# jeuneS2/csolve

Measured on AMD Instinct MI355X. Metric: constraint propagations/sec + nodes/sec, queens-N, 1/2/4/8 MI355X, higher is better.
Workload: dtype int32

## Files before the change

csolve_amd/_lib.py:

```python
from __future__ import annotations

import ctypes as C
import os
import re

_HERE = os.path.dirname(os.path.abspath(__file__))
LIB_PATH = os.environ.get("CSOLVE_HIP_LIB") or os.path.join(_HERE, "libcsolve_hip.so")
HEADER_PATH = os.path.join(os.path.dirname(_HERE), "include", "csolve_gpu.h")


class CsolveError(RuntimeError):
    def __init__(self, code: int, message: str):
        super().__init__(f"csolve_gpu error {code}: {message}")
        self.code = code


class Val(C.Structure):
    _fields_ = [("lo", C.c_int32), ("hi", C.c_int32)]


class Node(C.Structure):
    _fields_ = [("var", C.c_int32), ("lo", C.c_int32), ("hi", C.c_int32), ("parent", C.c_int32)]


# ... 173 lines not shown
    L.csgpu_search_drain_solutions_device.argtypes = [vp, vp, i64, C.POINTER(i64), vp]
    L.csgpu_search_pending_solutions.argtypes = [vp, C.POINTER(i64), C.POINTER(i64)]
    L.csgpu_propagate_one.argtypes = [vp, vp, Node, vp, C.POINTER(Result)]
    L.csgpu_propagate_one_traced.argtypes = [vp, vp, Node, vp, C.POINTER(Result), vp, i32, C.POINTER(i32)]
    L.csgpu_propagate_one_causes.argtypes = [vp, vp, Node, vp, C.POINTER(Result), vp, i32, C.POINTER(i32)]
    L.csgpu_propagate_values.argtypes = [vp, vp, i32, vp, i32, vp, vp]
    L.csgpu_model_root_propagate_limit.argtypes = [vp, i64, C.POINTER(i32), C.POINTER(i32)]
    L.csgpu_propagate_one_chain.argtypes = [vp, vp, Node, C.POINTER(i32), C.POINTER(i32), vp, i32, C.POINTER(i32)]
    L.csgpu_search_set_strategy.argtypes = [vp, C.c_int, C.c_int]
    L.csgpu_search_set_restart_on_improvement.argtypes = [vp, C.c_int]
    L.csgpu_internal_plan_symbol.argtypes = [vp, C.c_int, C.c_char_p, C.c_size_t]
    L.csgpu_solve_many.argtypes = [vp, vp, i64, C.POINTER(ManyOptions), vp, vp, vp]
    L.csgpu_internal_many_symbol.argtypes = [vp, C.c_char_p, C.c_size_t]
    L.csgpu_internal_many_waves.argtypes = [vp, i64]
    L.csgpu_internal_many_waves.restype = i64
    L.csgpu_internal_many_resume_symbol.argtypes = [vp, C.c_char_p, C.c_size_t]
    L.csgpu_many_checkpoint_bytes.argtypes = [vp]
    L.csgpu_many_checkpoint_bytes.restype = C.c_size_t
    L.csgpu_many_checkpoints_create.argtypes = [vp, i64, C.POINTER(vp)]
    L.csgpu_many_checkpoints_reset.argtypes = [vp, vp]
    L.csgpu_many_checkpoints_free.argtypes = [vp]
    L.csgpu_many_checkpoints_free.restype = None
    L.csgpu_solve_many_checkpointed.argtypes = [vp, vp, i64, C.POINTER(ManyOptions), vp, vp, vp, vp, vp]
    L.csgpu_solve_many_resume.argtypes = [vp, i64, C.POINTER(ManyOptions), vp, vp, vp, vp, vp]
    L.csgpu_many_checkpoint_states.argtypes = [vp, C.c_int32, vp, i64, C.POINTER(i64), vp]
    L.csgpu_solve_many_upto.argtypes = [vp, vp, i64, C.POINTER(ManyUptoOptions), vp, vp, vp]
    L.csgpu_solve_many_upto_checkpointed.argtypes = [vp, vp, i64, C.POINTER(ManyUptoOptions), vp, vp, vp, vp, vp]
    L.csgpu_solve_many_upto_resume.argtypes = [vp, i64, C.POINTER(ManyUptoOptions), vp, vp, vp, vp, vp]
    L.csgpu_internal_many_upto_symbol.argtypes = [vp, C.c_char_p, C.c_size_t]
    L.csgpu_solve_many_restarts.argtypes = [vp, vp, vp, i64, C.POINTER(ManyRestartOptions), vp, vp, vp, vp]
# ... 13 lines not shown
```

csolve_amd/csrc/cs_capi.hip:

```cpp
#include <hip/hip_runtime.h>
#include <chrono>

#include <dlfcn.h>
#include <stdarg.h>
#include <stdio.h>
#include <stdlib.h>
#include <string.h>

#include <mutex>

#include "../../include/csolve_gpu.h"
#include "cs_kernels.hip.h"
#include "cs_shave.hip.h"
#include "cs_step.hip.h"
#include "cs_dive.hip.h"
#include "cs_chain.hip.h"
#include "cs_internal.h"

static thread_local char g_err[512] = "";

static int set_err(int code, const char *fmt, ...) {
  va_list ap;
  va_start(ap, fmt);
  vsnprintf(g_err, sizeof g_err, fmt, ap);
// ... 50 lines not shown
  int not_root;
  int finalized;
  cs_dev_image *img;
  int *d_adj_off, *d_adj, *d_clause, *d_tree_off, *d_tnode, *d_tkid, *d_tree_want, *d_lit, *d_clause_by_kind;
  cs_tables tab;
  size_t slice;
  int has_tree_adj;
  int packed_bias;
  int packed_nw;
  int kernel_choice;
  cs_kernel_plan plan;
  void *d_adj_packed;
  int lds_adj_global;
  int k2_csz;
  int shave_static;
  int step_chunk_max;
  size_t k1_tab_bytes;
  int fb_words;
  size_t dense_bytes;
  void *d_dense_tab;
  void *d_packed_tab;
  int *d_root_lo;
  int *d_root_hi;
  void *d_many_stack;
  int64_t many_stack_waves;
  unsigned *d_many_tickets;
  int *d_sym_off;
  void *d_sym_packed;
  int n_cus;
  unsigned *d_tickets;
// ... 159 lines not shown
  (void)hipFree(m->d_lit);
  m->d_tree_want = NULL;
  m->d_lit = NULL;
  (void)hipFree(m->d_adj_packed);
  (void)hipFree(m->d_root_lo);
  (void)hipFree(m->d_root_hi);
  (void)hipFree(m->d_many_stack);
  (void)hipFree(m->d_many_tickets);
  m->d_root_hi = NULL;
  m->d_many_stack = NULL;
  m->d_many_tickets = NULL;
  m->many_stack_waves = 0;
  (void)hipFree(m->d_sym_off);
  (void)hipFree(m->d_sym_packed);
  (void)hipFree(m->d_dense_tab);
  (void)hipFree(m->d_packed_tab);
  m->d_packed_tab = NULL;
  (void)hipFree(m->d_tickets);
  m->d_tickets = NULL;
  m->ticket_slots = m->ticket_streams = m->ticket_reserved = 0;
  m->d_sym_off = NULL;
  m->d_sym_packed = NULL;
  m->d_dense_tab = NULL;
  m->d_adj_packed = NULL;
  m->d_root_lo = NULL;
  memset(&m->plan, 0, sizeof m->plan);
  m->fb_words = 0;
  (void)hipHostFree(m->h_one);
  m->h_one = NULL;
  (void)hipFree(m->d_adj_clause);
// ... 692 lines not shown
  const cs_model *h = m->host;
  if (!m->fb_words) return CSGPU_OK;
  const int n = h->n_vars, width = m->img->dense_width, slots = m->img->dense_slots;
  size_t bytes = 0;
  const int waves = dense_table_waves(m, &bytes);
  if (!waves) return CSGPU_OK;
  m->dense_bytes = bytes;
  int rc;
  if ((rc = upload(m->img->dense_tab, bytes, (int **)&m->d_dense_tab))) return rc;
  for (int variant = 0; variant < 4; variant++)
    if ((rc = plan_kernel(&m->plan.regs[variant], ne_regs_kernel(width, m->fb_words, n, variant & 1, variant >> 1), bytes, waves)))
      return rc;
  m->plan.full = n == cs_dense_strides(n) * CS_WAVE;
  if ((rc = plan_kernel(&m->plan.shave, ne_shave_kernel(width, n, slots, m->plan.full), bytes, waves))) return rc;
  const size_t table = (bytes + 15) & ~(size_t)15;
  if (table + (size_t)waves * 32 <= CS_CU_LDS &&
      (rc = plan_kernel(&m->plan.step_shave, step_shave_kernel(width, n, slots, m->plan.full), table + (size_t)waves * 32, waves)))
    return rc;
  if (table + CS_SHAVE_TRACE_LDS * 16 <= CS_CU_LDS) {
    if ((rc = plan_kernel(&m->plan.shave_trace, ne_shave_trace_kernel(width, n, slots), table + CS_SHAVE_TRACE_LDS * 16, waves)))
      return rc;
    m->plan.server = m->plan.shave_trace;
    m->plan.server.fn = shave_server_kernel(width, n, slots);
  }
  for (int family = 0; family < MANY_FAMILIES; family++)
    if ((rc = plan_kernel(&m->plan.dive[family], dive_kernel(family, width, n), table, waves))) return rc;
  {
    int *hi = (int *)malloc((size_t)n * sizeof(int));
    if (hi == NULL) return set_err(CSGPU_E_ARG, "out of memory");
    for (int32_t v = 0; v < n; v++) hi[v] = h->dom[v].hi;
// ... 131 lines not shown
  const void *fn = m->plan.dive[family].fn;
  const char *name = many_kernel_name[family];
  if (fn == NULL) return CSGPU_OK;
  Dl_info info;
  if (dladdr(fn, &info) == 0 || info.dli_sname == NULL || info.dli_saddr != fn)
    return set_err(CSGPU_E_STATE, "%s: the kernel handle has no dynamic symbol", name);
  if (strlen(info.dli_sname) >= len) return set_err(CSGPU_E_LIMIT, "%s: symbol longer than the buffer", name);
  strcpy(buf, info.dli_sname);
  return CSGPU_OK;
}

extern "C" int csgpu_internal_many_symbol(const csgpu_model *m, char *buf, size_t len) { return many_symbol(m, MANY_PLAIN, buf, len); }
extern "C" int csgpu_internal_many_resume_symbol(const csgpu_model *m, char *buf, size_t len) { return many_symbol(m, MANY_CK, buf, len); }
extern "C" int csgpu_internal_many_upto_symbol(const csgpu_model *m, char *buf, size_t len) { return many_symbol(m, MANY_UPTO, buf, len); }
extern "C" int csgpu_internal_many_restart_symbol(const csgpu_model *m, char *buf, size_t len) { return many_symbol(m, MANY_RESTART, buf, len); }

extern "C" void csgpu_internal_engine_ref(const csgpu_model *m, int delta) {
  if (m != NULL) const_cast<csgpu_model *>(m)->engines += delta;
}

extern "C" const int32_t *csgpu_internal_root_lo(const csgpu_model *m) {
  return m != NULL && m->finalized && m->fb_words ? m->d_root_lo : NULL;
}

extern "C" int csgpu_model_forbidden_words(const csgpu_model *m) { return m && m->finalized ? m->fb_words : 0; }

extern "C" int csgpu_internal_step_kind(const csgpu_model *m) { return m == NULL || !m->finalized ? 0 : m->plan.step_kind; }

static int64_t step_shave_waves(const csgpu_model *m, int64_t stage_rows) {
  const cs_planned *k = &m->plan.step_shave;
// ... 214 lines not shown
                        void *stream) {
  const cs_planned *k = &m->plan.shave;
  int csz = shrink_chunk(m->host->n_vars <= CS_WAVE ? 2 * CS_SHAVE_CHUNK : CS_SHAVE_CHUNK, batch, 4 * (int64_t)m->n_cus * 32);
  const int64_t chunks = (batch + csz - 1) / csz;
  int64_t g = (int64_t)m->n_cus * (int64_t)k->per_cu;
  const int64_t need_wg = (chunks + k->waves - 1) / k->waves;
  if (g > need_wg) g = need_wg;
  int n = m->host->n_vars, slots = m->img->dense_slots, dmin_d = m->img->dense_dmin;
  const void *tab_d = m->d_dense_tab;
  const int *root_lo_d = m->d_root_lo, *sym_off = m->d_sym_off;
  long long nb_d = (long long)batch;
  unsigned *tickets = m->shave_static ? NULL : ticket_slot((csgpu_model *)m, stream);
  int4 *no_trace = NULL;
  unsigned *no_trace_n = NULL;
  unsigned no_trace_cap = 0u;
  void *args[] = { &n, &tab_d, &slots, &dmin_d, &root_lo_d, &sym_off, &d_states_in, &d_nodes, &d_states_out, &d_results,
                   &nb_d, &d_batch, &csz, &tickets, &no_trace, &no_trace_n, &no_trace_cap };
  HIP_TRY(hipLaunchKernel(k->fn, dim3((unsigned)g), dim3((unsigned)(k->waves * CS_WAVE)), args, k->lds, (hipStream_t)stream));
  return CSGPU_OK;
}


static_assert(sizeof(csgpu_many_result) == sizeof(cs_dive_result) && sizeof(csgpu_many_result) == 40, "csgpu_many_result layout");
static_assert(sizeof(csgpu_many_restart_options) == 24, "csgpu_many_restart_options layout");

#define MANY_NOT_QUALIFIED "model does not qualify for the interval-only shaving kernel"

struct csgpu_many_checkpoints {
  const csgpu_model *m;
  int64_t capacity;
  size_t slot_bytes;
  cs_val *d_pool;
// ... 247 lines not shown
  if ((options->flags & ~CSGPU_MANY_ROTATE_FIRST) != 0) return set_err(CSGPU_E_ARG, "unknown flags 0x%x", (unsigned)options->flags);
  if ((rc = many_check_tail(m, MANY_RESTART, NULL, count))) return rc;
  cs_dive_rs rs;
  rs.seeds = d_seeds;
  rs.restarts = d_restarts;
  rs.restart_base = (long long)options->restart_base;
  rs.seed = options->seed;
  rs.flags = options->flags;
  return many_launch(m, MANY_RESTART, d_roots, count, options->max_nodes, 0, d_results, d_solutions, 0, stream, &rs, NULL);
}

#ifdef CS_SHAVE_TIMELINE
extern "C" int csgpu_debug_shave_timeline(unsigned long long *out, int waves) {
  HIP_TRY(hipDeviceSynchronize());
  HIP_TRY(hipMemcpyFromSymbol(out, HIP_SYMBOL(cs_shave_tl), (size_t)waves * 3 * sizeof(unsigned long long)));
  return CSGPU_OK;
}
#endif

extern "C" int csgpu_propagate_batch_fb(const csgpu_model *m, const csgpu_val *d_states_in, const uint64_t *d_forb_in,
                                        const csgpu_node *d_nodes, csgpu_val *d_states_out, uint64_t *d_forb_out,
                                        csgpu_result *d_results, int64_t batch, void *stream) {
  return csgpu_internal_propagate_fb(m, d_states_in, d_forb_in, d_nodes, d_states_out, d_forb_out, d_results, batch, NULL,
                                     stream);
}

extern "C" int csgpu_internal_propagate_fb(const csgpu_model *m, const csgpu_val *d_states_in, const uint64_t *d_forb_in,
                                           const csgpu_node *d_nodes, csgpu_val *d_states_out, uint64_t *d_forb_out,
                                           csgpu_result *d_results, int64_t batch, const uint64_t *d_batch,
                                           void *stream) {
// ... 498 lines not shown
  void *dev = NULL;
  HIP_TRY(hipHostGetDevicePointer(&dev, m->h_trace, 0));
  int4 *d_trace = (int4 *)dev;
  unsigned *d_trace_n = (unsigned *)((int32_t *)dev + (size_t)m->trace_cap * 4);
  unsigned ucap = (unsigned)cap;
  int n = m->host->n_vars, slots = m->img->dense_slots, dmin_d = m->img->dense_dmin, csz = 1;
  const void *tab_d = m->d_dense_tab;
  const int *root_lo_d = m->d_root_lo, *sym_off = m->d_sym_off;
  long long nb_d = 1;
  const uint64_t *d_batch = NULL;
  unsigned *tickets = NULL;
  const csgpu_val *d_in = (const csgpu_val *)m->d_one_in;
  const csgpu_node *d_node = (const csgpu_node *)m->d_one_node;
  csgpu_val *d_out = (csgpu_val *)m->d_one_out;
  csgpu_result *d_res = (csgpu_result *)m->d_one_res;
  void *args[] = { &n, &tab_d, &slots, &dmin_d, &root_lo_d, &sym_off, &d_in, &d_node, &d_out, &d_res,
                   &nb_d, &d_batch, &csz, &tickets, &d_trace, &d_trace_n, &ucap };
  const cs_planned *k = &m->plan.shave_trace;
  if (k->fn == NULL) return set_err(CSGPU_E_LIMIT, "no room in LDS for the trail next to the pair table");
  const double tl1 = srv_now();
  HIP_TRY(hipLaunchKernel(k->fn, dim3(1), dim3((unsigned)(k->waves * CS_WAVE)), args, k->lds, (hipStream_t)NULL));
  const double tl2 = srv_now();
  { const int rcw = wait_null_stream(); if (rcw != CSGPU_OK) return rcw; }
  const double tl3 = srv_now();
  memcpy(result, m->h_one + part + 64, sizeof *result);
  if (result->status >= 0) memcpy(state_out, m->h_one + part + 128, nbytes);
  const unsigned made = *m->h_trace_n;
  *count = (int32_t)made;
  unsigned kept = made < CS_SHAVE_TRACE_LDS ? made : CS_SHAVE_TRACE_LDS;
  if (kept > (unsigned)cap) kept = (unsigned)cap;
  memcpy(trace, m->h_trace, (size_t)kept * 16);
  m->srv_seconds[0] += tl1 - tl0; m->srv_seconds[1] += tl2 - tl1; m->srv_seconds[2] += tl3 - tl2; m->srv_seconds[3] += srv_now() - tl3;
// ... 104 lines not shown
```

csolve_amd/csrc/cs_device.c:

```c
#include "cs_device.h"

#include <stdio.h>
#include <stdlib.h>
#include <string.h>

#define NE_LIMIT (1 << 30)

typedef struct {
  int32_t *v;
  int32_t n, cap;
} ibuf;

static void ibuf_push(ibuf *b, int32_t x) {
  if (b->n == b->cap) {
    b->cap = b->cap ? b->cap * 2 : 256;
    b->v = (int32_t *)realloc(b->v, (size_t)b->cap * sizeof(int32_t));
    if (b->v == NULL) { fprintf(stderr, "csolve_amd: error: out of memory\n"); exit(EXIT_FAILURE); }
  }
  b->v[b->n++] = x;
}

static int small(int64_t x) { return x > -(int64_t)NE_LIMIT && x < (int64_t)NE_LIMIT; }

static int const_value(const cs_model *m, int32_t node, int64_t *c) {
// ... 125 lines not shown
    t->bad = 1;
    break;
  }
  int32_t idx = t->tnode.n / 4 - t->base;
  ibuf_push(&t->tnode, t->m->nodes[node].op);
  ibuf_push(&t->tnode, a);
  ibuf_push(&t->tnode, b);
  ibuf_push(&t->tnode, 0);
  t->local[node] = idx;
  ibuf_push(&t->touched, node);
  return idx;
}

void cs_dev_image_free(cs_dev_image *g) {
  if (g == NULL) return;
  free(g->adj_off); free(g->adj); free(g->adj_clause); free(g->clause); free(g->tree_off); free(g->tnode); free(g->tkid); free(g->tree_want); free(g->lit); free(g->adj_packed); free(g->sym_off); free(g->sym_packed); free(g->dense_tab);
  free(g);
}

cs_dev_image *cs_dev_image_build(const cs_model *m, int with_lists, const unsigned char *entailed, char *err,
                                 size_t errlen) {
  if (m->clause_node == NULL || (with_lists && m->list_off == NULL)) {
    if (err) snprintf(err, errlen, "model has no clause index");
    return NULL;
  }
  {
    const char *e = getenv("CSGPU_LINEAR_FAST_PATHS");
    if (e != NULL && e[0] == '0') cs_dev_linear_fast_paths = 0;
  }
  cs_dev_image *g = (cs_dev_image *)calloc(1, sizeof *g);
  g->n_vars = m->n_vars;
  g->n_clauses = m->n_clauses;
// ... 205 lines not shown
        memset(mult, 0, (size_t)n * (size_t)n);
        for (int32_t c = 0; c < g->n_clauses; c++) {
          const int32_t *rec = &g->clause[4 * c];
          if (rec[0] != CS_CL_NE) continue;
          const int k = mult[(size_t)rec[1] * n + rec[2]];
          mult[(size_t)rec[1] * n + rec[2]] = mult[(size_t)rec[2] * n + rec[1]] = (uint8_t)(k + 1);
          const uint32_t ea = (uint32_t)(rec[3] + m->dom[rec[2]].lo - dmin);
          const uint32_t eb = (uint32_t)(-rec[3] + m->dom[rec[1]].lo - dmin);
          const size_t ia = ((size_t)rec[1] * slots + k) * cols + rec[2];
          const size_t ib = ((size_t)rec[2] * slots + k) * cols + rec[1];
          if (dw == 1) { ((uint8_t *)g->dense_tab)[ia] = (uint8_t)ea; ((uint8_t *)g->dense_tab)[ib] = (uint8_t)eb; }
          else { ((uint16_t *)g->dense_tab)[ia] = (uint16_t)ea; ((uint16_t *)g->dense_tab)[ib] = (uint16_t)eb; }
        }
      }
      free(mult);
    }
  }
  return g;
}
```

csolve_amd/csrc/cs_device.h:

```cpp
#ifndef CS_DEVICE_H
#define CS_DEVICE_H

#include "cs_model.h"

#ifdef __cplusplus
extern "C" {
#endif

enum { CS_CL_SKIP = 0, CS_CL_NE = 1, CS_CL_TREE = 2, CS_CL_EQ = 3, CS_CL_LT = 4, CS_CL_OR2 = 5 };
enum { CS_REL_NE = 0, CS_REL_EQ = 1, CS_REL_LT = 2, CS_REL_GT = 3 };
#define CS_ADJ_VAR_MASK 0x0fffffff

static inline int cs_dense_strides(int32_t n_vars) { return n_vars <= 64 ? 1 : (n_vars <= 128 ? 2 : 4); }

#define CS_MAX_TREE_NODES 256

typedef struct cs_dev_image {
  int32_t n_vars, n_clauses;
  int32_t n_adj;
  int32_t n_ne, n_tree_clauses, n_skip;
  int32_t n_lin, n_or2;
  int32_t n_lits;
  int32_t *lit;
  int32_t max_list;
// ... 1 lines not shown
  int32_t *adj;
  int32_t *adj_clause;
  int32_t *clause;
  int32_t n_trees, n_tnodes, n_tkids, max_tree;
  int32_t *tree_off;
  int32_t *tnode;
  int32_t *tkid;
  int32_t *tree_want;
  int32_t packed_width, packed_obits, packed_dmin;
  void *adj_packed;
  int32_t sym_n_adj, sym_width, sym_obits, sym_dmin;
  int32_t *sym_off;
  void *sym_packed;
  int32_t dense_width, dense_slots, dense_cols, dense_dmin;
  void *dense_tab;
} cs_dev_image;

extern int cs_dev_linear_fast_paths;

cs_dev_image *cs_dev_image_build(const cs_model *m, int with_lists, const unsigned char *entailed, char *err,
                                 size_t errlen);
void cs_dev_image_free(cs_dev_image *img);

#ifdef __cplusplus
}
#endif
#endif
```

csolve_amd/csrc/cs_internal.h:

```cpp
#ifndef CS_INTERNAL_H
#define CS_INTERNAL_H

#include "../../include/csolve_gpu.h"
#include "cs_model.h"

#ifdef __cplusplus
extern "C" {
#endif

int csgpu_model_from_host(cs_model *host, int lists_final, int domains_are_root, csgpu_model **out);
cs_model *csgpu_model_host(csgpu_model *m);

int csgpu_internal_propagate_fb(const csgpu_model *m, const csgpu_val *d_states_in, const uint64_t *d_forb_in,
                                const csgpu_node *d_nodes, csgpu_val *d_states_out, uint64_t *d_forb_out,
                                csgpu_result *d_results, int64_t batch, const uint64_t *d_batch, void *stream);
int csgpu_internal_propagate_obj(const csgpu_model *m, const csgpu_val *d_states_in, const csgpu_node *d_nodes,
                                 csgpu_val *d_states_out, csgpu_result *d_results, int64_t batch,
                                 const uint64_t *d_batch, int32_t obj_lo, int32_t obj_hi, void *stream);

int csgpu_internal_propagate_objdev(const csgpu_model *m, const csgpu_val *d_states_in, const csgpu_node *d_nodes,
                                    csgpu_val *d_states_out, csgpu_result *d_results, int64_t batch,
                                    const uint64_t *d_batch, int32_t obj_lo, int32_t obj_hi, const int32_t *d_best,
                                    int sense, void *stream);
const int32_t *csgpu_internal_root_lo(const csgpu_model *m);
// ... 1 lines not shown
int csgpu_internal_eval_list(const csgpu_model *m, const csgpu_val *d_states, const int32_t *d_list,
                             const uint64_t *d_count, int64_t bound, int32_t *d_truth, void *stream);

int csgpu_internal_set_error(int code, const char *msg);
int csgpu_internal_search_info(const csgpu_search *s, int *objective, int *obj_var, int *n_vars, int *restarts,
                               int64_t *stream_rows);

int csgpu_internal_server_warm(csgpu_model *m);

int csgpu_internal_plan_symbol(const csgpu_model *m, int family, char *buf, size_t len);
int csgpu_internal_many_symbol(const csgpu_model *m, char *buf, size_t len);
int csgpu_internal_many_resume_symbol(const csgpu_model *m, char *buf, size_t len);
int csgpu_internal_many_upto_symbol(const csgpu_model *m, char *buf, size_t len);
int csgpu_internal_many_restart_symbol(const csgpu_model *m, char *buf, size_t len);
int64_t csgpu_internal_many_waves(const csgpu_model *m, int64_t count);

typedef struct csgpu_step_launch {
  const csgpu_val *pool;
  int64_t first_row;
  int32_t parents;
  csgpu_val *stage;
  int64_t stage_rows;
  uint32_t *fill;
  uint64_t *wstat;
  uint32_t *ticket;
  uint64_t *out;
  int32_t *solutions;
  uint64_t *stored;
  int64_t max_solutions;
  int32_t store_open;
// ... 19 lines not shown
```

csolve_amd/csrc/cs_shave.hip.h:

```cpp
#ifndef CS_SHAVE_HIP_H
#define CS_SHAVE_HIP_H

#include "cs_kernels.hip.h"

#ifdef CS_SHAVE_TIMELINE
__device__ unsigned long long cs_shave_tl[3 * 65536];
#endif

__device__ __forceinline__ unsigned long long cs_bitset0(unsigned long long m, int i) {
  asm("s_bitset0_b64 %0, %1" : "+s"(m) : "s"(i));
  return m;
}

__device__ __forceinline__ void cs_shift_if_eq(int &lo, int &hi, int f) {
  unsigned long long c;
  asm("v_cmp_eq_u32 vcc, %0, %3\n\t"
      "v_cmp_eq_u32 %2, %1, %3\n\t"
      "v_addc_co_u32 %0, vcc, 0, %0, vcc\n\t"
      "v_subb_co_u32 %1, %2, %1, 0, %2"
      : "+v"(lo), "+v"(hi), "=&s"(c) : "v"(f) : "vcc");
}
__device__ __forceinline__ void cs_shift_if_eq3(int &lo, int &hi, int f0, int f1, int f2) {
  unsigned long long c;
  asm("v_cmp_eq_u32 vcc, %0, %3\n\t"
// ... 23 lines not shown
__device__ __forceinline__ int cs_writelane(int v, int x) {
  x = __builtin_amdgcn_readfirstlane(x);
  asm("v_writelane_b32 %0, %1, %2" : "+v"(v) : "s"(x), "n"(L));
  return v;
}

__device__ __forceinline__ int cs_writelane_at(int lane, int v, int x) {
  switch (lane) {
  case 0: return cs_writelane<0>(v, x);
  case 1: return cs_writelane<1>(v, x);
  case 2: return cs_writelane<2>(v, x);
  default: return cs_writelane<3>(v, x);
  }
}

#define CS_SHAVE_TRACE_LDS 2048u
#define CS_SHAVE_CHUNK 2
#define CS_SHAVE_SHARDS 64
#define CS_SHAVE_TICKET_STRIDE 16

template <typename E, int R, int SL, bool TRACE>
struct cs_shave_core {
  typedef unsigned long long u64;
  static constexpr int W = CS_WAVE * R;
  const E *s_tab;
  int slots, lane;
  int kb[R], deg[R], b0[R];
  u64 livemask[R];
  int4 *s_trace;
  unsigned tcount;

  __device__ __forceinline__ void trace_lanes(u64 mask, int r2, int kind, int value, int cause) {
    if (mask == 0ull) return;
    const unsigned at = tcount + __builtin_amdgcn_mbcnt_hi((unsigned)(mask >> 32), __builtin_amdgcn_mbcnt_lo((unsigned)mask, 0u));
    if (__builtin_amdgcn_inverse_ballot_w64(mask) && at < CS_SHAVE_TRACE_LDS)
      s_trace[at] = make_int4(lane + r2 * CS_WAVE, kind, value + b0[r2], cause);
    tcount += (unsigned)__builtin_popcountll(mask);
  }

  __device__ __forceinline__ void push_var(int r, int ul, int cd, int (&rlo)[R], int (&rhi)[R], u64 (&dl)[R], u64 (&dh)[R],
                                           int &revisions) {
    revisions += __builtin_amdgcn_readlane(deg[r], ul);
    const E *row = s_tab + (size_t)(ul + r * CS_WAVE) * slots * W + lane;
    int plo[R], phi[R];
    if (TRACE) {
// ... 98 lines not shown
    } else {
      for (int k = 0; k < slots; k++) {
#pragma unroll
        for (int r2 = 0; r2 < R; r2++) {
          const u64 h = __ballot((int)row[k * W + r2 * CS_WAVE] == ckw - rlo[r2]) & val[r2];
          hit |= h;
          if (TRACE && CAUSE && cause < 0 && h != 0ull) cause = __builtin_ctzll(h) + r2 * CS_WAVE;
        }
      }
    }
    return hit;
  }

  template <int SIDE>
  __device__ __forceinline__ void verify_side(int (&rlo)[R], int (&rhi)[R], u64 (&dirty)[R], u64 (&val)[R], int &revisions,
                                              int &fail_v) {
#pragma unroll
    for (int r = 0; r < R; r++) {
      u64 bits = dirty[r];
      dirty[r] = 0ull;
      while (bits != 0ull) {
        const int wl = __builtin_ctzll(bits);
        bits = cs_bitset0(bits, wl);
        int cand = __builtin_amdgcn_readlane(SIDE == 0 ? rlo[r] : rhi[r], wl);
        const int ckw = cand + __builtin_amdgcn_readlane(kb[r], wl);
        revisions += __builtin_amdgcn_readlane(deg[r], wl);
        const E *row = s_tab + (size_t)(wl + r * CS_WAVE) * slots * W + lane;
        int e[SL ? SL : 1][R];
        if (SL != 0) {
#pragma unroll
          for (int k = 0; k < (SL ? SL : 1); k++)
#pragma unroll
            for (int r2 = 0; r2 < R; r2++) e[k][r2] = (int)row[k * W + r2 * CS_WAVE];
        }
        int cause = -1;
        if (forbidders<true>(row, e, ckw, rlo, val, cause) != 0ull) {
          const int other = __builtin_amdgcn_readlane(SIDE == 0 ? rhi[r] : rlo[r], wl);
          int step = 0;
          bool on;
          do {
            step++;
            on = SIDE == 0 ? cand + step <= other : cand - step >= other;
            if (on) on = forbidders<false>(row, e, ckw + (SIDE == 0 ? step : -step), rlo, val, cause) != 0ull;
          } while (on);
          cand += SIDE == 0 ? step : -step;
          if (lane == wl) { if (SIDE == 0) rlo[r] = cand; else rhi[r] = cand; }
          if (TRACE) trace_lanes(1ull << wl, r, SIDE, cand, cause);
          if (SIDE == 0 ? cand > other : cand < other) fail_v = wl + r * CS_WAVE;
          if (cand == other) val[r] |= 1ull << wl;
        }
      }
    }
  }

  __device__ __forceinline__ int round(int (&rlo)[R], int (&rhi)[R], u64 (&pushed)[R], u64 (&push)[R], u64 (&dl)[R],
                                       u64 (&dh)[R], u64 (&val)[R], int &revisions, bool &more) {
    more = false;
    push_phase(push, rlo, rhi, pushed, dl, dh, revisions);
    int fail_v = settle(rlo, rhi, val);
    if (fail_v < 0) {
      if (sweep_pays(dl, dh, val)) {
        bool again;
        do {
          u64 who[R];
#pragma unroll
          for (int r = 0; r < R; r++) { who[r] = val[r]; dl[r] = 0ull; dh[r] = 0ull; }
          push_phase(who, rlo, rhi, pushed, dl, dh, revisions);
          fail_v = settle(rlo, rhi, val);
          again = fail_v < 0;
          if (again) again = sweep_pays(dl, dh, val);
        } while (again);
      }
      if (fail_v < 0) {
        verify_side<0>(rlo, rhi, dl, val, revisions, fail_v);
        verify_side<1>(rlo, rhi, dh, val, revisions, fail_v);
        fail_v = __builtin_amdgcn_readfirstlane(fail_v);
        if (fail_v < 0) {
          u64 any_push = 0ull;
#pragma unroll
          for (int r = 0; r < R; r++) {
            push[r] = val[r] & ~pushed[r];
            any_push |= push[r];
          }
          more = any_push != 0ull;
        }
      }
    }
    return fail_v;
  }

// ... 17 lines not shown
      do {
        rounds++;
        fail_v = round(rlo, rhi, pushed, push, dl, dh, val, revisions, more);
      } while (more);
    }
    return fail_v;
  }
};

template <typename E, int R, int SL, bool FULL, bool TRACE = false>
__global__ __launch_bounds__(1024, (R <= 2 ? 8 : 4)) void cs_propagate_ne_shave(
    int n, const E *__restrict__ tab_g, int slots, int dmin, const int *__restrict__ root_lo,
    const int *__restrict__ sym_off, const cs_val *__restrict__ states_in, const cs_node_in *__restrict__ nodes,
    cs_val *__restrict__ states_out, cs_node_out *__restrict__ results, long long batch,
    const unsigned long long *__restrict__ batch_dev, int csz , unsigned *tickets,
    int4 *__restrict__ trace, unsigned *__restrict__ trace_n, unsigned trace_cap) {
  extern __shared__ __attribute__((aligned(16))) unsigned char cs_lds[];
  typedef unsigned long long u64;
  constexpr int W = CS_WAVE * R;
  constexpr int D = R == 1 && !TRACE ? 2 * CS_SHAVE_CHUNK : CS_SHAVE_CHUNK;
  if (batch_dev != nullptr && (long long)*batch_dev < batch) batch = (long long)*batch_dev;
  const int nbatch = __builtin_amdgcn_readfirstlane((int)batch);
  const int lane = threadIdx.x & (CS_WAVE - 1);
  const int wave_in_block = __builtin_amdgcn_readfirstlane(threadIdx.x >> 6);
  const int waves_per_block = blockDim.x >> 6;
  const int chunks = (nbatch + csz - 1) / csz;
  const int nsh = (int)gridDim.x < CS_SHAVE_SHARDS ? (int)gridDim.x : CS_SHAVE_SHARDS;
  const int shard = (int)(blockIdx.x % nsh);
  const int count_x = chunks > shard ? (chunks - 1 - shard) / nsh + 1 : 0;
  const int waves_x = (((int)gridDim.x - 1 - shard) / nsh + 1) * waves_per_block;
  const int wave_local = (int)(blockIdx.x / nsh) * waves_per_block + wave_in_block;
  const bool dynamic = tickets != nullptr && count_x > waves_x;
  if ((int)(blockIdx.x / nsh) * waves_per_block >= count_x) return;
  if (SL != 0) slots = SL;
  const E *s_tab = (const E *)cs_lds;
  int4 *s_trace = (int4 *)(cs_lds + ((((size_t)n * slots * W * sizeof(E)) + 15) & ~(size_t)15));
  {
    const int vecs = (int)(((size_t)n * slots * W * sizeof(E)) / 16);
    const uint4 *src = (const uint4 *)tab_g;
    uint4 *dst = (uint4 *)cs_lds;
    for (int i = threadIdx.x; i < vecs; i += blockDim.x) dst[i] = src[i];
  }
#ifdef CS_SHAVE_TIMELINE
  const unsigned long long tl_start = __builtin_amdgcn_s_memrealtime();
  unsigned long long tl_nodes = 0;
#endif
  __syncthreads();
  if (wave_local >= count_x) return;

  int b0[R], kb[R], deg[R], vcl[R];
  bool live[R];
#pragma unroll
  for (int r = 0; r < R; r++) {
    const int v = lane + r * CS_WAVE;
    live[r] = FULL || v < n;
    vcl[r] = live[r] ? v : n - 1;
    b0[r] = live[r] ? root_lo[vcl[r]] : 0;
    kb[r] = b0[r] - dmin;
    deg[r] = live[r] ? sym_off[vcl[r] + 1] - sym_off[vcl[r]] : 0;
  }
  u64 livemask[R];
#pragma unroll
  for (int r = 0; r < R; r++) livemask[r] = FULL ? ~0ull : __ballot(live[r]);
  cs_shave_core<E, R, SL, TRACE> C;
  C.s_tab = s_tab; C.slots = slots; C.lane = lane; C.s_trace = s_trace; C.tcount = 0u;
#pragma unroll
  for (int r = 0; r < R; r++) { C.kb[r] = kb[r]; C.deg[r] = deg[r]; C.b0[r] = b0[r]; C.livemask[r] = livemask[r]; }
  unsigned *my_ticket = tickets + (size_t)shard * CS_SHAVE_TICKET_STRIDE;

  auto load_rec = [&](int i) {
    cs_node_in rec;
    rec.var = -1; rec.lo = 0; rec.hi = 0; rec.parent = 0;
    const int node = (i * nsh + shard) * csz + lane;
    if (lane < csz && node < nbatch) rec = nodes[node];
    return rec;
  };
  auto next_index = [&](int i_prev, unsigned tk_v) -> int {
    if (!dynamic) return i_prev + waves_x;
    const int t = __builtin_amdgcn_readfirstlane((int)tk_v);
    if (t == count_x - 1 && lane == 0) __hip_atomic_store(my_ticket, 0u, __ATOMIC_RELAXED, __HIP_MEMORY_SCOPE_AGENT);
    return waves_x + t;
  };
// ... 118 lines not shown
    if (lane < cnt) results[base + lane] = my_result;

    if (!have_next) break;
    const int i_nn = next_index(i_next, tk);
    const int have_nn = i_nn < count_x;
    i_cur = i_next;
    rec_cur = rec_next;
#pragma unroll
    for (int d = 0; d < D; d++)
#pragma unroll
      for (int r = 0; r < R; r++) pd[d][r] = pn[d][r];
    rec_next = load_rec(have_nn ? i_nn : i_next);
    i_next = i_nn;
    have_next = have_nn;
  }
#ifdef CS_SHAVE_TIMELINE
  if (lane == 0) {
    const size_t w = ((size_t)blockIdx.x * (blockDim.x >> 6) + (threadIdx.x >> 6)) % 65536;
    cs_shave_tl[3 * w] = tl_start;
    cs_shave_tl[3 * w + 1] = __builtin_amdgcn_s_memrealtime();
    cs_shave_tl[3 * w + 2] = tl_nodes;
  }
#endif
}

struct cs_mailbox_head {
  unsigned req_seq; unsigned pad0[15];
  unsigned ack_seq; unsigned alive; unsigned pad1[14];
  unsigned stop; unsigned pad2[15];
  cs_node_in node; unsigned want_trace; unsigned pad3[11];
// ... 125 lines not shown
```

csolve_amd/solver.py:

```python
from __future__ import annotations

import contextlib
import ctypes as C

import numpy as np
import torch

from ._lib import (MANY_ROTATE_FIRST, PLAN_FAMILIES, CsolveError, ManyOptions, ManyRestartOptions, ManyResult,
                   ManyUptoOptions, Node, Result, SearchStats, Val, check, demangle, load_library)

STATUS_FAIL = -1


def _stream_ptr(stream) -> int:
    if stream is None:
        stream = torch.cuda.current_stream()
    return int(stream.cuda_stream)


class Model:

    def __init__(self, handle):
        self._h = handle
        self.finalized = False
# ... 113 lines not shown

    def set_kernel(self, which: int):
        check(load_library().csgpu_model_set_kernel(self._h, which))
        return self

    def qualifies(self, which: int) -> bool:
        return bool(load_library().csgpu_model_qualifies(self._h, which))

    def plan(self) -> dict:
        buf = C.create_string_buffer(1024)
        out = {}
        for i, fam in enumerate(PLAN_FAMILIES):
            check(load_library().csgpu_internal_plan_symbol(self._h, i, buf, len(buf)))
            out[fam] = demangle(buf.value.decode()) if buf.value else None
        return out

    def kernel(self) -> int:
        return check(load_library().csgpu_model_get_kernel(self._h))

    def root_state(self, device="cuda") -> torch.Tensor:
        return torch.from_numpy(self.domains()).to(device).unsqueeze(0).contiguous()

    def propagate(self, states_in: torch.Tensor, nodes: torch.Tensor, states_out: torch.Tensor = None,
                  results: torch.Tensor = None, stream=None):
        n = self.n_vars
        assert states_in.is_cuda and nodes.is_cuda, "device tensors required"
        assert states_in.dtype == torch.int32 and nodes.dtype == torch.int32
        assert states_in.is_contiguous() and nodes.is_contiguous()
        assert states_in.shape[-2:] == (n, 2) and nodes.shape[-1] == 4
        B = nodes.shape[0]
# ... 562 lines not shown
```

Baseline: 21.60 billion.

## Filter shaving verifications using detected not-equal offset groups in LDS flags

Detects, at model build time, groups of variables linked by all-different-with-offset not-equal constraints (as in queens diagonals) and computes per-variable base offsets into a small LDS flag region. In the shave kernel, before verifying dirty bounds, each wave marks fixed values in the flag region and skips verification of bounds whose candidate value collides with no fixed value in any group, restoring skipped lanes when a new value gets fixed. This targets redundant pairwise not-equal verification work, adjusting revision counts to stay consistent. It costs extra LDS per wave, extra flag writes and reads per round, and is only enabled when the extra LDS does not reduce residency.

```diff
diff --git a/csolve_amd/_lib.py b/csolve_amd/_lib.py
--- a/csolve_amd/_lib.py
+++ b/csolve_amd/_lib.py
@@ -211,6 +211,8 @@
     L.csgpu_internal_many_symbol.argtypes = [vp, C.c_char_p, C.c_size_t]
     L.csgpu_internal_many_waves.argtypes = [vp, i64]
     L.csgpu_internal_many_waves.restype = i64
+    if hasattr(L, "csgpu_internal_shave_groups"):
+        L.csgpu_internal_shave_groups.argtypes = [vp, C.POINTER(i32), C.POINTER(i32), C.POINTER(i32), C.POINTER(i32), vp, i64]
     L.csgpu_internal_many_resume_symbol.argtypes = [vp, C.c_char_p, C.c_size_t]
     L.csgpu_many_checkpoint_bytes.argtypes = [vp]
     L.csgpu_many_checkpoint_bytes.restype = C.c_size_t
diff --git a/csolve_amd/csrc/cs_capi.hip b/csolve_amd/csrc/cs_capi.hip
--- a/csolve_amd/csrc/cs_capi.hip
+++ b/csolve_amd/csrc/cs_capi.hip
@@ -88,6 +88,8 @@
   int lds_adj_global;
   int k2_csz;
   int shave_static;
+  int *d_shave_gbase;
+  int shave_gregion;
   int step_chunk_max;
   size_t k1_tab_bytes;
   int fb_words;
@@ -277,6 +279,9 @@
   (void)hipFree(m->d_sym_off);
   (void)hipFree(m->d_sym_packed);
   (void)hipFree(m->d_dense_tab);
+  (void)hipFree(m->d_shave_gbase);
+  m->d_shave_gbase = NULL;
+  m->shave_gregion = 0;
   (void)hipFree(m->d_packed_tab);
   m->d_packed_tab = NULL;
   (void)hipFree(m->d_tickets);
@@ -999,6 +1004,15 @@
   m->plan.full = n == cs_dense_strides(n) * CS_WAVE;
   if ((rc = plan_kernel(&m->plan.shave, ne_shave_kernel(width, n, slots, m->plan.full), bytes, waves))) return rc;
   const size_t table = (bytes + 15) & ~(size_t)15;
+  if (m->img->groups_on && cs_dense_strides(n) <= CS_SHAVE_FILTER_MAX_R) {
+    const size_t region = ((size_t)m->img->groups_region + 15) & ~(size_t)15;
+    const size_t with = table + (size_t)waves * region;
+    if (with <= CS_CU_LDS && resident_per_cu(with, waves) == m->plan.shave.per_cu) {
+      if ((rc = upload(m->img->groups_base, (size_t)slots * m->img->dense_cols * sizeof(int), &m->d_shave_gbase))) return rc;
+      if ((rc = plan_kernel(&m->plan.shave, m->plan.shave.fn, with, waves))) return rc;
+      m->shave_gregion = (int)region;
+    }
+  }
   if (table + (size_t)waves * 32 <= CS_CU_LDS &&
       (rc = plan_kernel(&m->plan.step_shave, step_shave_kernel(width, n, slots, m->plan.full), table + (size_t)waves * 32, waves)))
     return rc;
@@ -1160,6 +1174,22 @@
 extern "C" int csgpu_internal_many_resume_symbol(const csgpu_model *m, char *buf, size_t len) { return many_symbol(m, MANY_CK, buf, len); }
 extern "C" int csgpu_internal_many_upto_symbol(const csgpu_model *m, char *buf, size_t len) { return many_symbol(m, MANY_UPTO, buf, len); }
 extern "C" int csgpu_internal_many_restart_symbol(const csgpu_model *m, char *buf, size_t len) { return many_symbol(m, MANY_RESTART, buf, len); }
+
+extern "C" int csgpu_internal_shave_groups(const csgpu_model *m, int32_t *on, int32_t *region_bytes, int32_t *slots,
+                                           int32_t *cols, int32_t *bases, int64_t cap) {
+  if (m == NULL || on == NULL || region_bytes == NULL || slots == NULL || cols == NULL) return set_err(CSGPU_E_ARG, "null argument");
+  if (m->img == NULL) return set_err(CSGPU_E_STATE, "model has no device tables");
+  const cs_dev_image *g = m->img;
+  *on = g->groups_on;
+  *region_bytes = g->groups_region;
+  *slots = g->groups_region ? g->dense_slots : 0;
+  *cols = g->groups_region ? g->dense_cols : 0;
+  if (bases != NULL && g->groups_region) {
+    if (cap < (int64_t)g->dense_slots * g->dense_cols) return set_err(CSGPU_E_ARG, "room for %d bases needed", g->dense_slots * g->dense_cols);
+    memcpy(bases, g->groups_base, (size_t)g->dense_slots * g->dense_cols * sizeof(int32_t));
+  }
+  return CSGPU_OK;
+}
 
 extern "C" void csgpu_internal_engine_ref(const csgpu_model *m, int delta) {
   if (m != NULL) const_cast<csgpu_model *>(m)->engines += delta;
@@ -1404,8 +1434,10 @@
   int4 *no_trace = NULL;
   unsigned *no_trace_n = NULL;
   unsigned no_trace_cap = 0u;
+  const int *gbase = m->d_shave_gbase;
+  int gregion = m->shave_gregion, gwmax = m->img->groups_wmax;
   void *args[] = { &n, &tab_d, &slots, &dmin_d, &root_lo_d, &sym_off, &d_states_in, &d_nodes, &d_states_out, &d_results,
-                   &nb_d, &d_batch, &csz, &tickets, &no_trace, &no_trace_n, &no_trace_cap };
+                   &nb_d, &d_batch, &csz, &tickets, &no_trace, &no_trace_n, &no_trace_cap, &gbase, &gregion, &gwmax };
   HIP_TRY(hipLaunchKernel(k->fn, dim3((unsigned)g), dim3((unsigned)(k->waves * CS_WAVE)), args, k->lds, (hipStream_t)stream));
   return CSGPU_OK;
 }
@@ -1683,6 +1715,16 @@
 extern "C" int csgpu_debug_shave_timeline(unsigned long long *out, int waves) {
   HIP_TRY(hipDeviceSynchronize());
   HIP_TRY(hipMemcpyFromSymbol(out, HIP_SYMBOL(cs_shave_tl), (size_t)waves * 3 * sizeof(unsigned long long)));
+  return CSGPU_OK;
+}
+#endif
+
+#ifdef CS_SHAVE_FILTER_STATS
+extern "C" int csgpu_debug_shave_filter_stats(unsigned long long *out) {
+  static const unsigned long long zero[5] = { 0, 0, 0, 0, 0 };
+  HIP_TRY(hipDeviceSynchronize());
+  HIP_TRY(hipMemcpyFromSymbol(out, HIP_SYMBOL(cs_shave_fs), sizeof zero));
+  HIP_TRY(hipMemcpyToSymbol(HIP_SYMBOL(cs_shave_fs), zero, sizeof zero));
   return CSGPU_OK;
 }
 #endif
@@ -2211,8 +2253,10 @@
   const csgpu_node *d_node = (const csgpu_node *)m->d_one_node;
   csgpu_val *d_out = (csgpu_val *)m->d_one_out;
   csgpu_result *d_res = (csgpu_result *)m->d_one_res;
+  const int *no_gbase = NULL;
+  int no_gregion = 0, no_gwmax = 0;
   void *args[] = { &n, &tab_d, &slots, &dmin_d, &root_lo_d, &sym_off, &d_in, &d_node, &d_out, &d_res,
-                   &nb_d, &d_batch, &csz, &tickets, &d_trace, &d_trace_n, &ucap };
+                   &nb_d, &d_batch, &csz, &tickets, &d_trace, &d_trace_n, &ucap, &no_gbase, &no_gregion, &no_gwmax };
   const cs_planned *k = &m->plan.shave_trace;
   if (k->fn == NULL) return set_err(CSGPU_E_LIMIT, "no room in LDS for the trail next to the pair table");
   const double tl1 = srv_now();
diff --git a/csolve_amd/csrc/cs_device.c b/csolve_amd/csrc/cs_device.c
--- a/csolve_amd/csrc/cs_device.c
+++ b/csolve_amd/csrc/cs_device.c
@@ -163,8 +163,84 @@
 
 void cs_dev_image_free(cs_dev_image *g) {
   if (g == NULL) return;
-  free(g->adj_off); free(g->adj); free(g->adj_clause); free(g->clause); free(g->tree_off); free(g->tnode); free(g->tkid); free(g->tree_want); free(g->lit); free(g->adj_packed); free(g->sym_off); free(g->sym_packed); free(g->dense_tab);
+  free(g->adj_off); free(g->adj); free(g->adj_clause); free(g->clause); free(g->tree_off); free(g->tnode); free(g->tkid); free(g->tree_want); free(g->lit); free(g->adj_packed); free(g->sym_off); free(g->sym_packed); free(g->dense_tab); free(g->groups_base);
   free(g);
+}
+
+static void detect_groups(cs_dev_image *g, const cs_model *m) {
+  const int32_t n = m->n_vars, slots = g->dense_slots, cols = g->dense_cols;
+  if (g->dense_width == 0 || (slots != 1 && slots != 3) || n < 2 || cs_dense_strides(n) > 2) return;
+  for (int32_t v = 1; v < n; v++)
+    if (g->sym_off[v + 1] - g->sym_off[v] != g->sym_off[1] - g->sym_off[0]) return;
+  int64_t wmax = 0;
+  for (int32_t v = 0; v < n; v++)
+    if (m->dom[v].hi - m->dom[v].lo > wmax) wmax = m->dom[v].hi - m->dom[v].lo;
+  if (wmax >= CS_GROUPS_REGION_MAX) return;
+  const size_t nn = (size_t)n * (size_t)n;
+  int32_t *off = (int32_t *)calloc((size_t)slots * nn, sizeof(int32_t));
+  uint8_t *has = (uint8_t *)calloc((size_t)slots * nn, 1);
+  uint8_t *mult = (uint8_t *)calloc(nn, 1);
+  int64_t *t = (int64_t *)calloc((size_t)n, sizeof(int64_t));
+  int32_t *comp = (int32_t *)malloc((size_t)n * sizeof(int32_t));
+  uint8_t *seen = (uint8_t *)malloc((size_t)n);
+  int32_t *base = (int32_t *)malloc((size_t)slots * (size_t)cols * sizeof(int32_t));
+  for (int32_t c = 0; c < g->n_clauses; c++) {
+    const int32_t *rec = &g->clause[4 * c];
+    if (rec[0] != CS_CL_NE) continue;
+    const int k = mult[(size_t)rec[1] * n + rec[2]];
+    mult[(size_t)rec[1] * n + rec[2]] = mult[(size_t)rec[2] * n + rec[1]] = (uint8_t)(k + 1);
+    off[((size_t)k * n + rec[1]) * n + rec[2]] = rec[3];
+    off[((size_t)k * n + rec[2]) * n + rec[1]] = -rec[3];
+    has[((size_t)k * n + rec[1]) * n + rec[2]] = has[((size_t)k * n + rec[2]) * n + rec[1]] = 1;
+  }
+  int ok = 1;
+  int64_t total = 0;
+  for (int32_t i = 0; i < slots * cols; i++) base[i] = -1;
+  for (int32_t k = 0; k < slots && ok; k++) {
+    const int32_t *offk = off + (size_t)k * nn;
+    const uint8_t *hask = has + (size_t)k * nn;
+    memset(seen, 0, (size_t)n);
+    for (int32_t s = 0; s < n && ok; s++) {
+      if (seen[s]) continue;
+      seen[s] = 1;
+      int32_t len = 0;
+      comp[len++] = s;
+      t[s] = 0;
+      for (int32_t q = 0; q < len; q++) {
+        const int32_t u = comp[q];
+        for (int32_t w = 0; w < n; w++)
+          if (hask[(size_t)u * n + w] && !seen[w]) { seen[w] = 1; t[w] = t[u] + offk[(size_t)u * n + w]; comp[len++] = w; }
+      }
+      if (len == 1) continue;
+      int64_t kmin = m->dom[s].lo, kmax = m->dom[s].lo;
+      for (int32_t i = 0; i < len && ok; i++) {
+        const int32_t u = comp[i];
+        const int64_t key0 = m->dom[u].lo + t[u];
+        if (key0 < kmin) kmin = key0;
+        if (key0 > kmax) kmax = key0;
+        for (int32_t j = 0; j < len; j++) {
+          const int32_t w = comp[j];
+          if (w != u && (!hask[(size_t)u * n + w] || offk[(size_t)u * n + w] != t[w] - t[u])) { ok = 0; break; }
+        }
+      }
+      if (!ok || kmax + wmax - kmin + 1 > CS_GROUPS_REGION_MAX) { ok = 0; break; }
+      for (int32_t i = 0; i < len; i++)
+        base[(size_t)k * cols + comp[i]] = (int32_t)(total + m->dom[comp[i]].lo + t[comp[i]] - kmin);
+      total += kmax + wmax - kmin + 1;
+      if (total + wmax + 1 > CS_GROUPS_REGION_MAX) ok = 0;
+    }
+  }
+  if (ok && total > 0) {
+    for (int32_t i = 0; i < slots * cols; i++)
+      if (base[i] < 0) base[i] = (int32_t)total;
+    g->groups_region = (int32_t)(total + wmax + 1);
+    g->groups_wmax = (int32_t)wmax;
+    g->groups_base = base;
+    base = NULL;
+    const char *e = getenv("CSGPU_SHAVE_GROUPS");
+    g->groups_on = !(e != NULL && e[0] == '0');
+  }
+  free(base); free(seen); free(comp); free(t); free(mult); free(has); free(off);
 }
 
 cs_dev_image *cs_dev_image_build(const cs_model *m, int with_lists, const unsigned char *entailed, char *err,
@@ -400,6 +476,7 @@
         }
       }
       free(mult);
+      detect_groups(g, m);
     }
   }
   return g;
diff --git a/csolve_amd/csrc/cs_device.h b/csolve_amd/csrc/cs_device.h
--- a/csolve_amd/csrc/cs_device.h
+++ b/csolve_amd/csrc/cs_device.h
@@ -39,7 +39,11 @@
   void *sym_packed;
   int32_t dense_width, dense_slots, dense_cols, dense_dmin;
   void *dense_tab;
+  int32_t groups_region, groups_on, groups_wmax;
+  int32_t *groups_base;
 } cs_dev_image;
+
+#define CS_GROUPS_REGION_MAX 1024
 
 extern int cs_dev_linear_fast_paths;
 
diff --git a/csolve_amd/csrc/cs_internal.h b/csolve_amd/csrc/cs_internal.h
--- a/csolve_amd/csrc/cs_internal.h
+++ b/csolve_amd/csrc/cs_internal.h
@@ -39,6 +39,8 @@
 int csgpu_internal_many_upto_symbol(const csgpu_model *m, char *buf, size_t len);
 int csgpu_internal_many_restart_symbol(const csgpu_model *m, char *buf, size_t len);
 int64_t csgpu_internal_many_waves(const csgpu_model *m, int64_t count);
+int csgpu_internal_shave_groups(const csgpu_model *m, int32_t *on, int32_t *region_bytes, int32_t *slots, int32_t *cols,
+                                int32_t *bases, int64_t cap);
 
 typedef struct csgpu_step_launch {
   const csgpu_val *pool;
diff --git a/csolve_amd/csrc/cs_shave.hip.h b/csolve_amd/csrc/cs_shave.hip.h
--- a/csolve_amd/csrc/cs_shave.hip.h
+++ b/csolve_amd/csrc/cs_shave.hip.h
@@ -5,6 +5,9 @@
 
 #ifdef CS_SHAVE_TIMELINE
 __device__ unsigned long long cs_shave_tl[3 * 65536];
+#endif
+#ifdef CS_SHAVE_FILTER_STATS
+__device__ unsigned long long cs_shave_fs[5];
 #endif
 
 __device__ __forceinline__ unsigned long long cs_bitset0(unsigned long long m, int i) {
@@ -61,12 +64,14 @@
   }
 }
 
+typedef volatile __attribute__((address_space(3))) unsigned char cs_lds_flag;
+#define CS_SHAVE_FILTER_MAX_R 1
 #define CS_SHAVE_TRACE_LDS 2048u
 #define CS_SHAVE_CHUNK 2
 #define CS_SHAVE_SHARDS 64
 #define CS_SHAVE_TICKET_STRIDE 16
 
-template <typename E, int R, int SL, bool TRACE>
+template <typename E, int R, int SL, bool TRACE, bool FILTER = false>
 struct cs_shave_core {
   typedef unsigned long long u64;
   static constexpr int W = CS_WAVE * R;
@@ -76,6 +81,12 @@
   u64 livemask[R];
   int4 *s_trace;
   unsigned tcount;
+  bool groups;
+  int gb[SL ? SL : 1][R];
+  int gwmax, gdeg;
+#ifdef CS_SHAVE_FILTER_STATS
+  unsigned fs[5];
+#endif
 
   __device__ __forceinline__ void trace_lanes(u64 mask, int r2, int kind, int value, int cause) {
     if (mask == 0ull) return;
@@ -204,10 +215,10 @@
 
   template <int SIDE>
   __device__ __forceinline__ void verify_side(int (&rlo)[R], int (&rhi)[R], u64 (&dirty)[R], u64 (&val)[R], int &revisions,
-                                              int &fail_v) {
-#pragma unroll
-    for (int r = 0; r < R; r++) {
-      u64 bits = dirty[r];
+                                              int &fail_v, u64 (&skip)[R], u64 (&skip_next)[R]) {
+#pragma unroll
+    for (int r = 0; r < R; r++) {
+      u64 bits = FILTER ? dirty[r] & ~skip[r] : dirty[r];
       dirty[r] = 0ull;
       while (bits != 0ull) {
         const int wl = __builtin_ctzll(bits);
@@ -237,10 +248,94 @@
           if (lane == wl) { if (SIDE == 0) rlo[r] = cand; else rhi[r] = cand; }
           if (TRACE) trace_lanes(1ull << wl, r, SIDE, cand, cause);
           if (SIDE == 0 ? cand > other : cand < other) fail_v = wl + r * CS_WAVE;
+          const bool was_value = FILTER && ((val[r] >> wl) & 1ull) != 0ull;
           if (cand == other) val[r] |= 1ull << wl;
+          if (cand == other || was_value) {
+            if (FILTER) {
+              const u64 above = (~0ull << wl) << 1;
+              u64 back = skip[r] & above;
+              bits |= back;
+              skip[r] &= ~above;
+              int n_back = __builtin_popcountll(back);
+#pragma unroll
+              for (int r2 = 0; r2 < R; r2++) {
+                if (r2 > r) { n_back += __builtin_popcountll(skip[r2]); skip[r2] = 0ull; }
+                if (SIDE == 0) { n_back += __builtin_popcountll(skip_next[r2]); skip_next[r2] = 0ull; }
+              }
+              revisions -= gdeg * n_back;
+#ifdef CS_SHAVE_FILTER_STATS
+              fs[3] += (unsigned)n_back;
+              if (n_back != 0) fs[4]++;
+#endif
+            }
+          }
         }
       }
     }
+  }
+
+  __device__ __forceinline__ void filter(const int (&rlo)[R], const int (&rhi)[R], const u64 (&dl)[R], const u64 (&dh)[R],
+                                         const u64 (&val)[R], u64 (&skl)[R], u64 (&skh)[R], int &revisions) {
+    if (!groups) return;
+    constexpr int NS = SL ? SL : 1;
+    u64 any = 0ull;
+#pragma unroll
+    for (int r = 0; r < R; r++) any |= dl[r] | dh[r];
+    if (__builtin_expect(any == 0ull, 0)) return;
+    u64 bad = 0ull;
+    int cand[R];
+#pragma unroll
+    for (int r = 0; r < R; r++) {
+      cand[r] = __builtin_amdgcn_inverse_ballot_w64(dh[r]) ? rhi[r] : rlo[r];
+      bad |= __ballot((unsigned)cand[r] > (unsigned)gwmax);
+    }
+    if (__builtin_expect(bad != 0ull, 0)) {
+#ifdef CS_SHAVE_FILTER_STATS
+      fs[1]++;
+#endif
+      return;
+    }
+    cs_lds_flag *flag = (cs_lds_flag *)0u;
+    int a[NS][R];
+#pragma unroll
+    for (int k = 0; k < NS; k++)
+#pragma unroll
+      for (int r = 0; r < R; r++) a[k][r] = cand[r] + gb[k][r];
+#pragma unroll
+    for (int r = 0; r < R; r++)
+      if (__builtin_amdgcn_inverse_ballot_w64(val[r])) {
+#pragma unroll
+        for (int k = 0; k < NS; k++) flag[a[k][r]] = 1;
+      }
+    int seen[R];
+#pragma unroll
+    for (int r = 0; r < R; r++) {
+      seen[r] = 0;
+#pragma unroll
+      for (int k = 0; k < NS; k++) seen[r] |= flag[a[k][r]];
+    }
+#pragma unroll
+    for (int r = 0; r < R; r++)
+      if (__builtin_amdgcn_inverse_ballot_w64(val[r])) {
+#pragma unroll
+        for (int k = 0; k < NS; k++) flag[a[k][r]] = 0;
+      }
+    int n_skip = 0;
+#pragma unroll
+    for (int r = 0; r < R; r++) {
+      const u64 hit = __ballot(seen[r] != 0) | (dl[r] & dh[r]);
+      skl[r] = dl[r] & ~hit;
+      skh[r] = dh[r] & ~hit;
+      n_skip += __builtin_popcountll(skl[r] | skh[r]);
+#ifdef CS_SHAVE_FILTER_STATS
+      fs[2] += (unsigned)__builtin_popcountll(dl[r] | dh[r]);
+      fs[3] += (unsigned)__builtin_popcountll((dl[r] | dh[r]) & hit);
+#endif
+    }
+    revisions += gdeg * n_skip;
+#ifdef CS_SHAVE_FILTER_STATS
+    fs[0]++;
+#endif
   }
 
   __device__ __forceinline__ int round(int (&rlo)[R], int (&rhi)[R], u64 (&pushed)[R], u64 (&push)[R], u64 (&dl)[R],
@@ -262,8 +357,12 @@
         } while (again);
       }
       if (fail_v < 0) {
-        verify_side<0>(rlo, rhi, dl, val, revisions, fail_v);
-        verify_side<1>(rlo, rhi, dh, val, revisions, fail_v);
+        u64 skl[R], skh[R];
+#pragma unroll
+        for (int r = 0; r < R; r++) { skl[r] = 0ull; skh[r] = 0ull; }
+        if (FILTER) filter(rlo, rhi, dl, dh, val, skl, skh, revisions);
+        verify_side<0>(rlo, rhi, dl, val, revisions, fail_v, skl, skh);
+        verify_side<1>(rlo, rhi, dh, val, revisions, fail_v, skh, skl);
         fail_v = __builtin_amdgcn_readfirstlane(fail_v);
         if (fail_v < 0) {
           u64 any_push = 0ull;
@@ -311,10 +410,13 @@
     const int *__restrict__ sym_off, const cs_val *__restrict__ states_in, const cs_node_in *__restrict__ nodes,
     cs_val *__restrict__ states_out, cs_node_out *__restrict__ results, long long batch,
     const unsigned long long *__restrict__ batch_dev, int csz , unsigned *tickets,
-    int4 *__restrict__ trace, unsigned *__restrict__ trace_n, unsigned trace_cap) {
+    int4 *__restrict__ trace, unsigned *__restrict__ trace_n, unsigned trace_cap,
+    const int *__restrict__ gbase , int gregion ,
+    int gwmax) {
   extern __shared__ __attribute__((aligned(16))) unsigned char cs_lds[];
   typedef unsigned long long u64;
   constexpr int W = CS_WAVE * R;
+  constexpr bool FILTER = !TRACE && R <= CS_SHAVE_FILTER_MAX_R && (SL == 1 || SL == 3);
   constexpr int D = R == 1 && !TRACE ? 2 * CS_SHAVE_CHUNK : CS_SHAVE_CHUNK;
   if (batch_dev != nullptr && (long long)*batch_dev < batch) batch = (long long)*batch_dev;
   const int nbatch = __builtin_amdgcn_readfirstlane((int)batch);
@@ -338,6 +440,11 @@
     uint4 *dst = (uint4 *)cs_lds;
     for (int i = threadIdx.x; i < vecs; i += blockDim.x) dst[i] = src[i];
   }
+  const int flags0 = (int)((((size_t)n * slots * W * sizeof(E)) + 15) & ~(size_t)15);
+  if (FILTER && gbase != nullptr) {
+    unsigned *dst = (unsigned *)(cs_lds + flags0);
+    for (int i = threadIdx.x; i < waves_per_block * gregion / 4; i += blockDim.x) dst[i] = 0u;
+  }
 #ifdef CS_SHAVE_TIMELINE
   const unsigned long long tl_start = __builtin_amdgcn_s_memrealtime();
   unsigned long long tl_nodes = 0;
@@ -359,10 +466,22 @@
   u64 livemask[R];
 #pragma unroll
   for (int r = 0; r < R; r++) livemask[r] = FULL ? ~0ull : __ballot(live[r]);
-  cs_shave_core<E, R, SL, TRACE> C;
+  cs_shave_core<E, R, SL, TRACE, FILTER> C;
   C.s_tab = s_tab; C.slots = slots; C.lane = lane; C.s_trace = s_trace; C.tcount = 0u;
 #pragma unroll
   for (int r = 0; r < R; r++) { C.kb[r] = kb[r]; C.deg[r] = deg[r]; C.b0[r] = b0[r]; C.livemask[r] = livemask[r]; }
+  C.groups = FILTER && gbase != nullptr;
+  const int lds0 = (int)(unsigned)(unsigned long)(cs_lds_flag *)cs_lds;
+  C.gwmax = gwmax;
+  C.gdeg = __builtin_amdgcn_readfirstlane(deg[0]);
+#pragma unroll
+  for (int k = 0; k < (SL ? SL : 1); k++)
+#pragma unroll
+    for (int r = 0; r < R; r++)
+      C.gb[k][r] = C.groups ? gbase[k * W + lane + r * CS_WAVE] + lds0 + flags0 + wave_in_block * gregion : 0;
+#ifdef CS_SHAVE_FILTER_STATS
+  for (int i = 0; i < 5; i++) C.fs[i] = 0u;
+#endif
   unsigned *my_ticket = tickets + (size_t)shard * CS_SHAVE_TICKET_STRIDE;
 
   auto load_rec = [&](int i) {
@@ -511,6 +630,10 @@
     i_next = i_nn;
     have_next = have_nn;
   }
+#ifdef CS_SHAVE_FILTER_STATS
+  if (lane == 0)
+    for (int i = 0; i < 5; i++) atomicAdd(&cs_shave_fs[i], (unsigned long long)C.fs[i]);
+#endif
 #ifdef CS_SHAVE_TIMELINE
   if (lane == 0) {
     const size_t w = ((size_t)blockIdx.x * (blockDim.x >> 6) + (threadIdx.x >> 6)) % 65536;
diff --git a/csolve_amd/solver.py b/csolve_amd/solver.py
--- a/csolve_amd/solver.py
+++ b/csolve_amd/solver.py
@@ -151,6 +151,17 @@
             check(load_library().csgpu_internal_plan_symbol(self._h, i, buf, len(buf)))
             out[fam] = demangle(buf.value.decode()) if buf.value else None
         return out
+
+    def shave_groups(self) -> dict:
+        on, region, slots, cols = C.c_int32(), C.c_int32(), C.c_int32(), C.c_int32()
+        L = load_library()
+        check(L.csgpu_internal_shave_groups(self._h, C.byref(on), C.byref(region), C.byref(slots), C.byref(cols), None, 0))
+        bases = None
+        if region.value:
+            bases = np.empty((slots.value, cols.value), dtype=np.int32)
+            check(L.csgpu_internal_shave_groups(self._h, C.byref(on), C.byref(region), C.byref(slots), C.byref(cols),
+                                                bases.ctypes.data, bases.size))
+        return {"on": bool(on.value), "region_bytes": region.value, "bases": bases}
 
     def kernel(self) -> int:
         return check(load_library().csgpu_model_get_kernel(self._h))
```

Result: no change. 21.63 billion (median of 4 runs) (+0.1%).
